# zhengchen1999/DOVE

Hardware: AMD Instinct MI355X
Metric: SR frames/s (33x720x1280 4x one-step, whole job) (higher is better)
Workload: dtype bf16; 1 GPU; synthetic 33x720x1280 HR clip (LR 180x320, 4x), one-step t=399, CogVideoX1.5-5B VAE + 42-layer DiT random-init, 1 clip per GPU (BASELINE configs[1]); weight_sums=True, vae_streams=2, variant=headline (bf16)

## Files before the change

### dove_amd/csrc/igemm.hip

```cpp
#include "igemm_args.h"


template <int BN, int BK>
struct FastCfg {
  static constexpr int BM = 128;
  static constexpr int CPR = BK / 8;
  static constexpr int CPR_LOG = (BK == 64) ? 3 : 2;
  static constexpr int RPG = 256 / CPR;
  static constexpr int NA = BM / RPG;
  static constexpr int B_SLOTS = BN * CPR;
  static constexpr int NB = (B_SLOTS + 255) / 256;
  static constexpr int A_BYTES = BM * BK * 2, B_BYTES = BN * BK * 2, STAGE = A_BYTES + B_BYTES;
  static constexpr int WN = (BN >= 128) ? 2 : 1, WM = 4 / WN;
  static constexpr int PT = (BM / WM) / 32, CT = (BN / WN) / 32;
  static constexpr int KK = BK / 16;
};

template <int BN, int BK>
__global__ __launch_bounds__(256) void igemm_fast_kernel(const IgemmArgs a) {
  using Cf = FastCfg<BN, BK>;
  constexpr int NA = Cf::NA, NB = Cf::NB, PT = Cf::PT, CT = Cf::CT, KK = Cf::KK, STAGE = Cf::STAGE, A_BYTES = Cf::A_BYTES;
  extern __shared__ __attribute__((aligned(16))) char smem[];
  const int tid = threadIdx.x, lane = tid & 63;
  const int wave = __builtin_amdgcn_readfirstlane(tid >> 6);
// ... 1053 lines not shown
#pragma unroll 4
  for (int r = 0; r < smallk::ROWS; ++r) {
    const long long m = r0 + r;
    if (m >= M) break;
    uint32_t xr[16];
#pragma unroll
    for (int q = 0; q < 4; ++q) {
      const uint4 v = xs[wave * smallk::ROWS + r][q];
      xr[q * 4 + 0] = v.x; xr[q * 4 + 1] = v.y; xr[q * 4 + 2] = v.z; xr[q * 4 + 3] = v.w;
    }
    float acc[4] = {b[0], b[1], b[2], b[3]};
#pragma unroll
    for (int k = 0; k < 16; ++k)
#pragma unroll
      for (int j = 0; j < 4; ++j)
        acc[j] = __builtin_amdgcn_fdot2_f32_bf16(__builtin_bit_cast(v2bf, wr[j][k]), __builtin_bit_cast(v2bf, xr[k]), acc[j], false);
    uint2 o;
    o.x = pack_bf2(acc[0], acc[1]);
    o.y = pack_bf2(acc[2], acc[3]);
    *(uint2*)(out + m * ldo + n0) = o;
  }
}

enum ConvKernel { K_IGEMM = 0, K_IGEMM_FAST, K_HALO4X, K_HALO4X_UP, K_GEMM8P, K_SMALLK, K_HALO4X_SUB };
static const char* const kKernelNames[] = {"igemm_kernel", "igemm_fast_kernel", "conv3x3_halo4x_kernel", "conv3x3_halo4x_kernel", "gemm8p_kernel",
                                           "smallk_kernel", "conv3x3_halo4x_kernel"};

static inline int desc_nb(const dove_conv_desc* d) { return d->nb > 1 ? d->nb : 1; }

static ConvKernel select_kernel(const dove_conv_desc* d) {
  const long long M = (long long)desc_nb(d) * d->t_out * d->h_out * d->w_out;
  const bool frame_fits = (long long)d->h_in * d->w_in * d->cin * 2 < (1ll << 31);
  const bool plain_gemm = d->kt == 1 && d->kh == 1 && d->kw == 1 && d->stride == 1 && d->up == 0 && d->tmode == 0 &&
                          d->t_in == d->t_out && d->h_in == d->h_out && d->w_in == d->w_out && d->cout_pad % 128 == 0 && M >= 4096 &&
                          (long long)512 * d->cin * 2 < (1ll << 31);
  const bool pointwise = d->kt == 1 && d->kh == 1 && d->kw == 1 && d->stride == 1 && d->up == 0 && d->tmode == 0 && d->t_in == d->t_out &&
                         d->h_in == d->h_out && d->w_in == d->w_out;
  if (pointwise && d->cin == 32 && d->act == 0 && !d->resid && !d->gate && d->cout_store >= 128) return K_SMALLK;
  if (plain_gemm) {
    if (d->cout_pad % 256 == 0 && d->cout_store % 256 == 0 && d->cin % 128 == 0 && d->cin >= 256 && (long long)256 * d->cin * 2 < (1ll << 31) &&
        d->ldo < (1 << 20) && d->ldr < (1 << 20) && (d->act == 0 || d->act == 1))
      return K_GEMM8P;
  }
  const bool conv3 = d->kh == 3 && d->kw == 3 && d->stride == 1 && d->pad_h == 1 && d->pad_w == 1 && d->act == 0 && !d->gate &&
                     d->cout_pad % 128 == 0 && frame_fits;
  if (conv3) {
    const bool same = d->up == 0 && d->tmode == 0 && d->h_out == d->h_in && d->w_out == d->w_in && d->w_out >= 16 && d->h_out >= 16;
    const bool ups = d->up == 1 && d->kt == 1 && d->h_out == 2 * d->h_in && d->w_out == 2 * d->w_in && d->h_out >= 16 && d->w_out >= 32;
    const bool h4 = d->cout_store % 128 == 0 && d->cin % 64 == 0 && d->ldo < (1 << 20) && (!d->resid || d->ldr < (1 << 20));
    if (same && h4) return K_HALO4X;
    if (ups && h4 && d->w_sub && d->h_in >= 16 && d->w_in >= 32) return K_HALO4X_SUB;
    if (ups && h4) return K_HALO4X_UP;
  }
  const int BN = (d->cout_pad % 128 == 0) ? 128 : ((d->cout_pad % 64 == 0) ? 64 : 32);
  const bool fits = frame_fits && (long long)BN * d->cin * 2 < (1ll << 31);
  return (d->up == 0 && fits) ? K_IGEMM_FAST : K_IGEMM;
}

static bool desc_size_ok(const dove_conv_desc* d, const char* who) {
  if (d && d->struct_size == sizeof(dove_conv_desc) && d->reserved == 0) return true;
  if (d) dove_set_error("%s: dove_conv_desc.struct_size is %u, this library (ABI %d) expects %zu - the caller's binding was written "
                        "against another include/dove_hip.h", who, d->struct_size, DOVE_ABI_VERSION, sizeof(dove_conv_desc));
  else dove_set_error("%s: null descriptor", who);
  return false;
}
extern "C" const char* dove_conv_kernel_name(const dove_conv_desc* d) { return desc_size_ok(d, "conv_kernel_name") ? kKernelNames[select_kernel(d)] : ""; }

template <int BN, int BK>
static int launch_igemm_fast(const IgemmArgs& a, unsigned grid, hipStream_t s) {
  constexpr int lds = 2 * (128 * BK * 2 + BN * BK * 2);
  static PerDeviceOnce attr_set;
  if (auto once_ = attr_set.guard()) (void)hipFuncSetAttribute((const void*)igemm_fast_kernel<BN, BK>, hipFuncAttributeMaxDynamicSharedMemorySize, lds);
  hipLaunchKernelGGL((igemm_fast_kernel<BN, BK>), dim3(grid), dim3(256), lds, s, a);
  DOVE_CHECK_LAUNCH("dove_conv_igemm_bf16");
  return DOVE_OK;
}
// ... 62 lines not shown
  DOVE_CHECK_ARG(d->x && d->w && d->out, "conv_igemm: null pointer");
  DOVE_CHECK_ARG(d->cin % 32 == 0 && d->cin > 0, "conv_igemm: Cin (%d) must be a positive multiple of 32 (pad on pack)", d->cin);
  DOVE_CHECK_ARG(d->cout_pad % 32 == 0 && d->cout_pad > 0, "conv_igemm: Cout_pad (%d) must be a multiple of 32", d->cout_pad);
  DOVE_CHECK_ARG(d->cout_store % 4 == 0 && d->cout_store <= d->cout_pad && d->cout_store > 0, "conv_igemm: bad cout_store %d", d->cout_store);
  DOVE_CHECK_ARG(d->ldo % 4 == 0 && d->ldo >= d->cout_store, "conv_igemm: ldo (%lld) must be a multiple of 4 and >= cout_store", d->ldo);
  DOVE_CHECK_ARG(!d->resid || (d->ldr % 4 == 0 && d->ldr >= d->cout_store), "conv_igemm: bad ldr %lld", d->ldr);
  DOVE_CHECK_ARG(!d->gate || d->resid, "conv_igemm: gate needs resid");
  DOVE_CHECK_ARG(d->kt >= 1 && d->kt <= 3 && d->kh >= 1 && d->kw >= 1, "conv_igemm: bad kernel size");
  DOVE_CHECK_ARG(d->stride == 1 || d->stride == 2, "conv_igemm: stride must be 1 or 2");
  DOVE_CHECK_ARG(d->up == 0 || d->up == 1, "conv_igemm: up must be 0/1");
  DOVE_CHECK_ARG(d->kt == 1 || (d->tmode == 0 && d->t_in == d->t_out), "conv_igemm: causal temporal taps need t_in == t_out and tmode 0");
  DOVE_CHECK_ARG(d->t_out > 0 && d->h_out > 0 && d->w_out > 0 && d->t_in > 0 && d->h_in > 0 && d->w_in > 0, "conv_igemm: empty tensor");
  DOVE_CHECK_ARG(d->nb >= 0 && d->nb <= 4096 && (long long)desc_nb(d) * d->t_out < (1 << 20), "conv_igemm: bad instance count nb = %d", d->nb);
  DOVE_CHECK_ARG(d->cache_stride == 0 || (d->cache && d->cache_stride >= (long long)(d->kt - 1) * d->h_in * d->w_in * d->cin),
                 "conv_igemm: cache_stride (%lld) is smaller than one instance's cache", d->cache_stride);
  DOVE_CHECK_ARG(desc_nb(d) == 1 || !d->gate, "conv_igemm: nb > 1 is not combined with gate");
  DOVE_CHECK_ARG(d->reserved2 == 0 && d->tdup >= 0 && d->tdup <= 2, "conv_igemm: bad tdup %d", d->tdup);
  DOVE_CHECK_ARG(!d->tdup || (d->kt == 3 && d->w_pair), "conv_igemm: tdup declares frame pairs of a kt == 3 conv and needs w_pair");
  DOVE_CHECK_ARG(!d->tdup || d->cache || d->w_first, "conv_igemm: tdup without a conv cache needs w_first too (frames whose three taps read one frame)");
  DOVE_CHECK_ARG(d->tdup != 2 || !d->cache, "conv_igemm: tdup == 2 (first frame single) is the head of a clip: no conv cache");
  DOVE_CHECK_ARG(!d->gn_partial || dove_conv_gn_partial_rows(d) > 0,
                 "conv_igemm: gn_partial requested but this call does not dispatch to a kernel that fuses the statistics");
  const ConvKernel kern0 = select_kernel(d);
  DOVE_CHECK_ARG(!d->out_f32 || (kern0 == K_IGEMM_FAST && !d->resid && d->act == 0),
                 "conv_igemm: out_f32 is only implemented for plain convs that dispatch to igemm_fast_kernel");
  long long rows_main = 0;
  if (kern0 == K_GEMM8P && gemm_tail_split(d, &rows_main)) {
    dove_conv_desc m = *d, t = *d;
    m.w_in = m.w_out = (int)rows_main;
    const long long tail = (long long)d->w_out - rows_main;
    t.w_in = t.w_out = (int)tail;
    t.x = (const char*)d->x + rows_main * d->cin * 2;
    t.out = (char*)d->out + rows_main * d->ldo * 2;
    if (d->resid) t.resid = (const char*)d->resid + rows_main * d->ldr * 2;
    t.gate_split = d->gate_split > rows_main ? d->gate_split - rows_main : 0;
    const int rc = conv_dispatch(&m, stream, K_GEMM8P);
    return rc ? rc : conv_dispatch(&t, stream, K_IGEMM_FAST);
  }
  return conv_dispatch(d, stream, kern0);
}

static int conv_dispatch(const dove_conv_desc* d, void* stream, ConvKernel kern) {
  const bf16_t* zp = zero_page();
  DOVE_CHECK_ARG(zp, "conv_igemm: could not allocate the zero page");
  IgemmArgs a;
  a.x = (const bf16_t*)d->x; a.cache = (const bf16_t*)d->cache; a.w = (const bf16_t*)d->w;
  a.bias = d->bias; a.resid = (const bf16_t*)d->resid; a.gate = d->gate; a.out = (bf16_t*)d->out; a.zero = zp;
  const int nb = desc_nb(d);
  a.T_out = nb * d->t_out; a.H_out = d->h_out; a.W_out = d->w_out;
  a.T_in = nb * d->t_in; a.H_in = d->h_in; a.W_in = d->w_in;
  a.seg_out = d->t_out; a.seg_in = d->t_in;
  a.cache_bs = d->cache_stride ? d->cache_stride : (long long)(d->kt - 1) * d->h_in * d->w_in * d->cin;
  a.Cin = d->cin; a.Cout_pad = d->cout_pad; a.Cout_st = d->cout_store;
  a.kt = d->kt; a.kh = d->kh; a.kw = d->kw; a.stride = d->stride; a.pad_h = d->pad_h; a.pad_w = d->pad_w;
  a.up = d->up; a.tmode = d->tmode; a.act = d->act; a.ldo = d->ldo; a.ldr = d->ldr; a.gate_split = d->gate_split;
  a.gn_partial = nullptr; a.cpg_log = 0;
  a.w_first = nullptr;
  a.w_pair = nullptr; a.tdup = 0;
  a.sub = 0;
  a.out_f32 = d->out_f32;
  a.nt_out = 0;
  a.reserved = 0;
  hipStream_t s = (hipStream_t)stream;
  const long long M = (long long)nb * d->t_out * d->h_out * d->w_out;
  switch (kern) {
    case K_GEMM8P: {
      a.tiles_n = d->cout_pad / 256;
      a.nt_out = (long long)M * d->ldo * 2 > (256ll << 20);
      const long long nt = ((M + gemm4x::BM - 1) / gemm4x::BM) * a.tiles_n;
      DOVE_CHECK_ARG(nt > 0 && nt < (1ll << 31), "conv_igemm: grid too large");
      DOVE_CHECK_ARG(!(d->gate && d->act), "conv_igemm: gate with activation is not a path of the reference");
      const int cus = cu_count();
      const unsigned grid4 = nt > cus ? (unsigned)cus : (unsigned)nt;
      static PerDeviceOnce attr8;
      if (auto once_ = attr8.guard()) {
        (void)hipFuncSetAttribute((const void*)gemm8p_kernel<false, false>, hipFuncAttributeMaxDynamicSharedMemorySize, gemm8p::LDS_BYTES);
        (void)hipFuncSetAttribute((const void*)gemm8p_kernel<true, false>, hipFuncAttributeMaxDynamicSharedMemorySize, gemm8p::LDS_BYTES);
        (void)hipFuncSetAttribute((const void*)gemm8p_kernel<false, true>, hipFuncAttributeMaxDynamicSharedMemorySize, gemm8p::LDS_BYTES);
      }
      if (d->gate) hipLaunchKernelGGL((gemm8p_kernel<false, true>), dim3(grid4), dim3(512), gemm8p::LDS_BYTES, s, a, M);
      else if (d->act == 1) hipLaunchKernelGGL((gemm8p_kernel<true, false>), dim3(grid4), dim3(512), gemm8p::LDS_BYTES, s, a, M);
      else hipLaunchKernelGGL((gemm8p_kernel<false, false>), dim3(grid4), dim3(512), gemm8p::LDS_BYTES, s, a, M);
      DOVE_CHECK_LAUNCH("dove_conv_igemm_bf16(gemm8p)");
      return DOVE_OK;
    }
    case K_SMALLK: {
      dim3 grid((unsigned)((M + 4 * smallk::ROWS - 1) / (4 * smallk::ROWS)), (unsigned)((d->cout_store + 255) / 256));
      hipLaunchKernelGGL(smallk_kernel, grid, dim3(256), 0, s, a.x, a.w, a.bias, a.out, M, d->cout_store, d->ldo);
// ... 86 lines not shown
```

### dove_amd/csrc/igemm_args.h

```cpp
#pragma once
#include <stdlib.h>

#include <type_traits>

#include "common.h"
#include "../../include/dove_hip.h"

struct IgemmArgs {
  const bf16_t* x;
  const bf16_t* cache;
  const bf16_t* w;
  const float* bias;
  const bf16_t* resid;
  const float* gate;
  bf16_t* out;
  const bf16_t* zero;
  int T_out, H_out, W_out;
  int T_in, H_in, W_in;
  int Cin, Cout_pad, Cout_st;
  int kt, kh, kw, stride, pad_h, pad_w, up, tmode, act;
  long long ldo, ldr;
  long long gate_split;
  int tw_log2, tiles_w, tiles_h, tiles_n;
  int reserved;
// ... 51 lines not shown
  q.m0 = __builtin_amdgcn_readfirstlane((int)(group * GM + within % gm) * gemm4x::BM);
  q.n0 = __builtin_amdgcn_readfirstlane((int)(within / gm) * gemm4x::BN);
  return q;
}
__device__ __forceinline__ void g4_open_tile(G4State& s, const IgemmArgs& a, const G4Const& k, int id) {
  s.n_tile = id;
  s.n_on = id < k.ntiles;
  const G4Tile q = g4_decode(k, id);
  const long long left = k.M - q.m0;
  const int rows = left < gemm4x::BM ? (int)left : gemm4x::BM;
  s.a_base = a.x + (long long)q.m0 * k.K;
  s.w_base = a.w + (long long)q.n0 * k.K;
  s.a_nrec = s.n_on ? rows * k.K * 2 : 0;
  s.w_nrec = s.n_on ? gemm4x::BN * k.K * 2 : 0;
  s.n_k4 = 0;
  s.soff = 0;
}
__device__ __forceinline__ void g4_advance(G4State& s, const IgemmArgs& a, const G4Const& k) {
  if (++s.n_k4 == k.nk4) g4_open_tile(s, a, k, s.n_tile + k.G);
  s.soff = s.n_k4 * (4 * gemm4x::ROWB);
}

int launch_igemm_legacy(const IgemmArgs& a, unsigned grid, int BN, bool bk64, hipStream_t s);
```

### dove_amd/lib.py

```python
from __future__ import annotations

import ctypes as C
import os

import torch

_HERE = os.path.dirname(os.path.abspath(__file__))
LIB_PATH = os.path.join(_HERE, "libdove_hip.so")
_lib = None

F32, BF16, U8 = 0, 1, 2
METRIC_PSNR, METRIC_SSIM, METRIC_RGB_TO_Y = 1, 2, 4
COLORFIX_WAVELET, COLORFIX_ADAIN, COLORFIX_CLAMP = 1, 2, 1
YUV_444, YUV_422, YUV_420, YUV_MONO = 0, 1, 2, 3
YUV_SITING_LEFT, YUV_SITING_CENTRE = 0, 1
VIDEO_RGB_U8, VIDEO_YUV = 0, 1
RESIZE_BILINEAR, RESIZE_BICUBIC, RESIZE_AREA = 0, 1, 2
ACT_NONE, ACT_RELU, ACT_SIGMOID, ACT_TANH = 0, 1, 2, 3


class ConvDesc(C.Structure):
    _fields_ = [
        ("struct_size", C.c_uint), ("reserved", C.c_uint),
        ("x", C.c_void_p), ("cache", C.c_void_p), ("w", C.c_void_p), ("bias", C.c_void_p),
# ... 90 lines not shown
                ("stride", C.c_int), ("pool", C.c_int), ("relu", C.c_int), ("reserved2", C.c_int),
                ("ldx", C.c_longlong), ("ldr", C.c_longlong), ("ldo", C.c_longlong)]

    def __init__(self, *a, **k):
        super().__init__(*a, **k)
        self.struct_size = C.sizeof(ResnetConvF32Args)


class PreNoise(C.Structure):
    _fields_ = [("eps", C.c_void_p), ("eps_dtype", C.c_int), ("sqrt_alpha", C.c_float), ("sqrt_one_minus_alpha", C.c_float)]


OPT_VAE_TILING, OPT_VAE_SAMPLE_HEIGHT, OPT_VAE_SAMPLE_WIDTH, OPT_DIT_LINEAR_MXFP8, OPT_DIT_ATTN_MXFP8, OPT_WEIGHT_SUMS, OPT_VAE_STREAMS = 1, 2, 3, 4, 5, 6, 7
STAT_HALO_PREPOSTED, STAT_HALO_BLOCKING, STAT_HALO_SENT, STAT_HALO_COMMUNICATORS = 100, 101, 102, 103


_VP, _I, _LL, _F = C.c_void_p, C.c_int, C.c_longlong, C.c_float
_ULL, _PI, _PLL = C.c_ulonglong, C.POINTER(C.c_int), C.POINTER(C.c_longlong)
XFER_FN = C.CFUNCTYPE(C.c_int, C.c_void_p, C.c_int, C.c_void_p, C.c_size_t, C.c_void_p)
GROUP_FN = C.CFUNCTYPE(C.c_int, C.c_void_p, C.c_void_p)

SIGNATURES = {
    "dove_conv_igemm_bf16": [C.POINTER(ConvDesc), _VP],
    "dove_groupnorm_stats_bf16": [_VP, _LL, _LL, _I, _F, _VP, _I, _VP, _VP],
    "dove_groupnorm_finalize_partials": [_VP, _LL, C.c_double, _F, _VP, _VP, _VP],
    "dove_groupnorm_stats_nb_bf16": [_VP, _I, _LL, _LL, _I, _F, _VP, _I, _VP, _VP],
    "dove_groupnorm_finalize_partials_nb": [_VP, _LL, _I, C.c_double, _F, _VP, C.c_size_t, _VP, _VP],
    "dove_groupnorm_apply_nb_bf16": [_VP, _VP, _I, _I, _I, _I, _I, _VP, _VP, _VP, _I, _VP, _I, _I, _I, _I, C.POINTER(C.c_int), _VP],
    "dove_avgpool_time_nb_bf16": [_VP, _I, _I, _LL, _VP, _VP],
    "dove_groupnorm_sums_bf16": [_VP, _LL, _LL, _I, _VP, _I, _VP, _VP],
    "dove_groupnorm_finalize_sums": [_VP, C.c_double, _F, _VP, _VP],
    "dove_groupnorm_sums_from_partials": [_VP, _LL, _VP, _VP, _VP],
    "dove_groupnorm_apply_bf16": [_VP, _VP, _I, _I, _I, _I, _VP, _VP, _VP, _I, _VP, _I, _I, _I, C.POINTER(C.c_int), _VP],
    "dove_layernorm_modulate_bf16": [_VP, _VP, _LL, _I, _F, _VP, _VP, _VP, _LL, _VP],
    "dove_qkv_post_bf16": [_VP, _LL, _LL, _I, _I, _I, _VP, _VP, _VP, _VP, _VP, _VP, _F, _F, _VP, _VP, _VP, _I, _VP, _VP],
    "dove_vt_quad_swap_bf16": [_VP, _LL, _LL, _VP],
    "dove_ulysses_place_bf16": [_VP, _VP, _VP, C.POINTER(C.c_longlong), _I, _I, _LL, _LL, _VP, _VP, _VP, _VP, _VP],
    "dove_cl_im2col3x3_from_ncthw": [_VP, _I, _I, _I, _I, _I, _I, _F, _F, _VP, _VP],
    "dove_conv_out_gather": [_VP, _LL, _I, _I, _I, _I, _VP, _F, _F, _F, _F, _VP, _I, _VP],
    "dove_attention_fwd_bf16": [_VP, _VP, _VP, _VP, _LL, _LL, _I, _I, _LL, _VP, _VP],
    "dove_qkv_post_mxfp8": [_VP, _LL, _LL, _I, _I, _I, _VP, _VP, _VP, _VP, _VP, _VP, _F, _F, _VP, _VP, _VP, _VP, _VP],
    "dove_attention_fwd_mxfp8": [_VP, _VP, _VP, _VP, _VP, _LL, _LL, _I, _I, _LL, _VP],
    "dove_cl_from_ncthw": [_VP, _I, _I, _LL, _I, _F, _F, _VP, _VP],
    "dove_ncthw_from_cl": [_VP, _LL, _I, _LL, _F, _F, _F, _F, _VP, _I, _VP],
    "dove_avgpool_time_bf16": [_VP, _I, _LL, _VP, _VP],
    "dove_posterior_sample": [_VP, _LL, _I, _LL, _VP, _I, _VP, _I, _VP],
# ... 91 lines not shown
    "dove_swin3d_window_gather_f32": [_VP, _I, _PI, _I, _PI, _PI, _VP, _VP],
    "dove_swin3d_window_scatter_f32": [_VP, _VP, _I, _PI, _I, _PI, _PI, _VP, _VP],
    "dove_swin3d_patch_merge_f32": [_VP, _LL, _I, _I, _I, _VP, _VP],
    "dove_swin3d_window_attention_f32": [_VP, _VP, _VP, _LL, _LL, _I, _I, _F, _VP, _VP, _I, _VP, _VP, _VP, _I, _VP, _LL, _VP],
    "dove_vqa_head_f64": [_VP, _LL, _I, _I, _I, _VP, _VP, _I, _VP, _VP, _VP, _VP],
    "dove_dwconv3d_f32": [_VP, _I, _I, _I, _I, _I, _VP, _VP, _VP, _VP],
    "dove_vqa_resized_view_f32": [C.POINTER(ImageView), _I, _I, _I, _VP, _I, _VP, _VP, _I, _VP, _VP, _I, _I, _I, C.POINTER(C.c_double),
                                  C.POINTER(C.c_double), _I, _VP, _VP],
    "dove_bmm_f32": [_VP, _LL, _LL, _VP, _LL, _LL, _VP, _VP, _LL, _LL, _VP, _LL, _LL, _I, _I, _I, _I, _F, _I, _VP],
    "dove_softmax_rows_f32": [_VP, _LL, _LL, _I, _VP, _LL, _VP],
    "dove_window_attention_f32": [_VP, _VP, _VP, _LL, _LL, _I, _I, _I, _F, _VP, _I, _VP, _VP, _I, _VP, _LL, _VP],
    "dove_maniqa_crops_f32": [C.POINTER(ImageView), _I, _I, _I, _I, _VP, _I, _I, _I, _VP, _VP],
    "dove_maniqa_tokens_f32": [_VP, _VP, _VP, _LL, _I, _I, _VP, _VP],
    "dove_mix_f32": [_VP, _LL, _LL, _VP, _LL, _LL, _F, _I, _I, _I, _I, _VP, _LL, _LL, _VP],
    "dove_maniqa_score": [_VP, _LL, _I, _I, _I, _I, _VP, _VP, _VP, _VP, _VP, _VP, _VP],
    "dove_png_encode": [C.POINTER(ImageView), _I, _I, _I, _I, _VP, C.c_size_t, _VP, _VP, _VP],
    "dove_zlib_huffman": [_VP, _LL, _LL, _VP, C.c_size_t, _VP, _VP, _VP],
    "dove_jpeg_encode": [C.POINTER(ImageView), _I, _I, _I, C.POINTER(C.c_int), _I, _VP, C.c_size_t, _VP, _VP, _VP],
}
PLAIN = {"dove_last_error": (C.c_char_p, []), "dove_abi_version": (C.c_int, []), "dove_comm_destroy": (None, [C.c_void_p]),
         "dove_conv_gn_partial_rows": (C.c_longlong, [C.POINTER(ConvDesc)]),
         "dove_conv_kernel_name": (C.c_char_p, [C.POINTER(ConvDesc)]),
         "dove_conv_partial_launches": (C.c_int, [C.POINTER(ConvDesc)]),
         "dove_attention_head_paths": (C.c_int, [C.POINTER(C.c_float), _I, C.POINTER(C.c_int)]),
         "dove_attention_path_name": (C.c_char_p, [_I]),
         "dove_device_info": (C.c_int, [_I, C.c_char_p, _I, C.POINTER(C.c_int), C.POINTER(C.c_longlong)]),
         "dove_destroy": (None, [_VP]),
         "dove_vae_decode_num_frames": (C.c_int, [_VP, _I]),
         "dove_get_option": (C.c_longlong, [_VP, _I]),
         "dove_comm_useful_ranks": (C.c_int, [_VP, _I, _I]),
         "dove_workspace_bytes": (C.c_size_t, [_VP, _I, _I, _I]),
         "dove_workspace_high_water": (C.c_size_t, [_VP]),
         "dove_fr_metrics_workspace_bytes": (C.c_size_t, [_I, _I, _I]),
         "dove_color_fix_workspace_bytes": (C.c_size_t, [_I, _I, _I, _I]),
         "dove_yuv_frame_bytes": (C.c_size_t, [_I, _I, _I]),
         "dove_poisson_noise_workspace_bytes": (C.c_size_t, [_I]),
         "dove_jpeg_roundtrip_workspace_bytes": (C.c_size_t, [_I, _I, _I]),
         "dove_vcodec_workspace_bytes": (C.c_size_t, [_I, _I, _I, _I]),
         "dove_vcodec_tools_workspace_bytes": (C.c_size_t, [_I, _I, _I, _I, _I]),
         "dove_chunk_planner_need": (C.c_longlong, [_VP]),
         "dove_chunk_planner_destroy": (None, [_VP]),
         "dove_video_workspace_bytes": (C.c_size_t, [_VP, C.POINTER(VideoParams)]),
         "dove_video_close": (None, [_VP]),
         "dove_instance_norm_f32_workspace_bytes": (C.c_size_t, [_I, _I, _I, _I]),
         "dove_flow_warp_error_workspace_bytes": (C.c_size_t, [_I, _I, _I]),
         "dove_convnet_conv_f32_kernel_name": (C.c_char_p, [C.POINTER(ConvnetConvF32Args)]),
# ... 90 lines not shown
```

### dove_amd/ops.py

```python
from __future__ import annotations

import ctypes as C
import math
from dataclasses import dataclass

import numpy as np
import torch

from . import lib as L


def _ru(x: int, m: int) -> int:
    return (x + m - 1) // m * m


@dataclass
class PackedConv:
    w: torch.Tensor
    bias: torch.Tensor | None
    kt: int
    kh: int
    kw: int
    cin: int
    cin_pad: int
# ... 55 lines not shown
        return [("w012", 0)] if tl == 0 else [("w01", 0), ("w2", 1)]
    if tdup == 1:
        if not cached and tl < 2:
            return [("w012", tl)]
        return [("w0", tl - 2), ("w12", tl)] if tl & 1 else [("w01", tl - 1), ("w2", tl)]
    if tl == 0:
        return [("w012", 0)]
    return [("w01", tl - 1), ("w2", tl)] if tl & 1 else [("w0", tl - 2), ("w12", tl)]


def temporal_groups(tl: int, tdup: int, cached: bool) -> int:
    return len(temporal_split(tl, tdup, cached))


_profiler = None


def set_profiler(records: list | None):
    global _profiler
    _profiler = records


def conv_kernel_name(x_shape, pc: PackedConv, *, stride=1, pad=(None, None), up=0, tmode=0, t_out=None, hw_out=None, act=0, gated=False,
                     resid=False, nb=1, partial=False):
    T, H, W, Cx = x_shape
    d = L.ConvDesc()
    d.nb = nb
    ph = (pc.kh - 1) // 2 if pad[0] is None else pad[0]
    pw = (pc.kw - 1) // 2 if pad[1] is None else pad[1]
    t_out = T if t_out is None else t_out
    if hw_out is None:
        hw_out = (H << up, W << up) if stride == 1 else ((H + 1 - pc.kh) // stride + 1, (W + 1 - pc.kw) // stride + 1)
    d.t_in, d.h_in, d.w_in, d.cin = T, H, W, Cx
    d.t_out, d.h_out, d.w_out = t_out, hw_out[0], hw_out[1]
    d.cout_pad, d.cout_store = pc.cout_pad, pc.cout_store
    d.kt, d.kh, d.kw, d.stride, d.pad_h, d.pad_w = pc.kt, pc.kh, pc.kw, stride, ph, pw
    d.up, d.tmode, d.act = up, tmode, act
    d.ldo = pc.cout_store
    d.ldr = pc.cout_store if resid else 0
    d.resid = 1 if (resid or gated) else None
    d.w_sub = 1 if (up == 1 and pc.kt == 1 and pc.kh == 3 and pc.kw == 3) else None
    d.gate = 1 if gated else None
    if partial:
        return int(L.load().dove_conv_partial_launches(C.byref(d)))
    return L.load().dove_conv_kernel_name(C.byref(d)).decode()


def conv(x: torch.Tensor, pc: PackedConv, *, cache: torch.Tensor | None = None, stride: int = 1, pad=(None, None),
         up: int = 0, tmode: int = 0, t_out: int | None = None, hw_out=None, resid: torch.Tensor | None = None,
         gate: torch.Tensor | None = None, gate_split: int = 0, act: int = 0, ldo: int | None = None,
         out: torch.Tensor | None = None,
         gn_eps: float | None = None, out_f32: bool = False, nb: int = 1, tdup: int = 0, weight_sums: bool = True) -> torch.Tensor:
    L.require_cuda(x, resid, gate, out)
    assert x.dtype == torch.bfloat16 and x.dim() == 4, (x.dtype, x.shape)
    T, H, W, Cx = x.shape
    assert T % nb == 0, (T, nb)
    T //= nb
    if Cx != pc.cin_pad:
        raise RuntimeError(f"conv: input has {Cx} channels, packed weight expects {pc.cin_pad}")
    ph = (pc.kh - 1) // 2 if pad[0] is None else pad[0]
    pw = (pc.kw - 1) // 2 if pad[1] is None else pad[1]
    if t_out is None:
        t_out = T
    if hw_out is None:
        hw_out = (H << up, W << up) if stride == 1 else ((H + 1 - pc.kh) // stride + 1, (W + 1 - pc.kw) // stride + 1)
    if ldo is None:
        ldo = pc.cout_store
    odt = torch.float32 if out_f32 else torch.bfloat16
    if out is None:
        out = torch.empty(nb * t_out, hw_out[0], hw_out[1], ldo, dtype=odt, device=x.device)
    else:
        assert out.shape == (nb * t_out, hw_out[0], hw_out[1], ldo) and out.dtype == odt
    cache_stride = 0
    if cache is not None:
        if nb > 1:
# ... 18 lines not shown
    d.out = out.data_ptr()
    d.t_in, d.h_in, d.w_in, d.cin = T, H, W, Cx
    d.t_out, d.h_out, d.w_out = t_out, hw_out[0], hw_out[1]
    d.cout_pad, d.cout_store = pc.cout_pad, pc.cout_store
    d.kt, d.kh, d.kw, d.stride, d.pad_h, d.pad_w = pc.kt, pc.kh, pc.kw, stride, ph, pw
    d.up, d.tmode, d.act = up, tmode, act
    d.ldo = ldo
    d.ldr = resid.shape[-1] if resid is not None else 0
    d.gate_split = gate_split
    d.out_f32 = int(out_f32)
    if resid is not None:
        assert resid.dtype == torch.bfloat16 and resid.numel() == nb * t_out * hw_out[0] * hw_out[1] * resid.shape[-1]
    if gate is not None:
        assert gate.dtype == torch.float32 and gate.shape == (2, pc.cout_pad)
    partial = None
    if gn_eps is not None and ldo == pc.cout_store:
        rows = int(L.load().dove_conv_gn_partial_rows(C.byref(d)))
        if rows > 0:
            partial = torch.empty(rows, 64, dtype=torch.float32, device=x.device)
            d.gn_partial = partial.data_ptr()
    if _profiler is not None:
        e0, e1 = torch.cuda.Event(enable_timing=True), torch.cuda.Event(enable_timing=True)
        e0.record()
    L.check(L.load().dove_conv_igemm_bf16(C.byref(d), L.stream_ptr()), "dove_conv_igemm_bf16")
    if _profiler is not None:
        e1.record()
        flops = 2.0 * nb * t_out * hw_out[0] * hw_out[1] * pc.cout * pc.cin * pc.kt * pc.kh * pc.kw
        name = L.load().dove_conv_kernel_name(C.byref(d)).decode()
        real = flops
        if name == "conv3x3_halo4x_kernel":
            if d.tdup and pc.kt == 3 and up == 0:
                real = flops * sum(temporal_groups(tl, d.tdup, cache is not None) for tl in range(t_out)) / (3.0 * t_out)
            elif d.w_first and pc.kt == 3 and up == 0:
                real = flops * (1.0 - (2.0 + (1.0 if t_out > 1 else 0.0)) / (3.0 * t_out))
            elif d.w_sub and up == 1 and H >= 16 and W >= 32:
                real = flops * 4.0 / 9.0
        _profiler.append(((pc.cin, pc.cout, pc.kt * pc.kh * pc.kw), flops, e0, e1, name, real))
    if partial is None:
        if getattr(out, "gn_stats", None) is not None:
            out.gn_stats = None
            out.gn_rows = None
    else:
        count = float(t_out * hw_out[0] * hw_out[1]) * (pc.cout_store // 32)
        if nb > 1:
            stats = torch.empty(nb, 32, 2, dtype=torch.float32, device=x.device)
            ws = _ws(x.device, nb * 512)
            L.check(L.load().dove_groupnorm_finalize_partials_nb(partial.data_ptr(), partial.shape[0] // nb, nb, count, gn_eps, L.ptr(ws),
                                                                 ws.numel() * 4, L.ptr(stats), L.stream_ptr()), "dove_groupnorm_finalize_partials_nb")
        else:
            stats = torch.empty(32, 2, dtype=torch.float32, device=x.device)
            L.check(L.load().dove_groupnorm_finalize_partials(partial.data_ptr(), partial.shape[0], count, gn_eps, L.ptr(_ws(x.device)),
# ... 1638 lines not shown
```

### include/dove_hip.h

```cpp
#ifndef DOVE_HIP_H
#define DOVE_HIP_H

#include <stddef.h>

#ifdef __cplusplus
extern "C" {
#endif

#define DOVE_ABI_VERSION 15

#define DOVE_F32 0
#define DOVE_BF16 1

const char* dove_last_error(void);
int dove_abi_version(void);
int dove_device_info(int dev, char* name, int name_len, int* cu_count, long long* total_mem);

typedef struct dove_conv_desc {
  unsigned int struct_size;
  unsigned int reserved;
  const void* x;
  const void* cache;
  const void* w;
  const float* bias;
  const void* resid;
  const float* gate;
  void* out;
  int t_in, h_in, w_in, cin;
  int t_out, h_out, w_out, cout_pad, cout_store;
  int kt, kh, kw, stride, pad_h, pad_w, up, tmode, act;
  long long ldo, ldr, gate_split;
  float* gn_partial;
  int out_f32;
  int nb;
  long long cache_stride;
  const void* w_first;
  const void* w_sub;
  const void* w_pair;
  int tdup;
  int reserved2;
} dove_conv_desc;
int dove_conv_igemm_bf16(const dove_conv_desc* d, void* stream);
const char* dove_conv_kernel_name(const dove_conv_desc* d);
int dove_conv_partial_launches(const dove_conv_desc* d);
long long dove_conv_gn_partial_rows(const dove_conv_desc* d);
int dove_groupnorm_finalize_partials(const float* partial, long long rows, double count, float eps, void* ws, float* stats,
                                     void* stream);

int dove_groupnorm_stats_bf16(const void* x, long long npix, long long frame_pix, int C, float eps, void* partial_ws, int ws_blocks,
                              float* stats, void* stream);
int dove_groupnorm_sums_bf16(const void* x, long long npix, long long frame_pix, int C, void* partial_ws, int ws_blocks, double* sums,
                             void* stream);
int dove_groupnorm_finalize_sums(const double* sums, double count, float eps, float* stats, void* stream);
int dove_groupnorm_sums_from_partials(const float* partial, long long rows, void* ws, double* sums, void* stream);
int dove_groupnorm_apply_bf16(const void* x, void* y, int T, int H, int W, int C, const float* stats,
                              const float* gamma, const float* beta, int silu, const void* yb, int hz, int wz,
                              int sshift, const int* tmap, void* stream);

int dove_groupnorm_stats_nb_bf16(const void* x, int nb, long long npix, long long frame_pix, int C, float eps, void* partial_ws,
                                 int ws_blocks, float* stats, void* stream);
int dove_groupnorm_finalize_partials_nb(const float* partial, long long rows, int nb, double count, float eps, void* ws, size_t ws_bytes,
                                        float* stats, void* stream);
int dove_groupnorm_apply_nb_bf16(const void* x, void* y, int nb, int T, int H, int W, int C, const float* stats, const float* gamma,
                                 const float* beta, int silu, const void* yb, int Tz, int hz, int wz, int sshift, const int* tmap,
                                 void* stream);
int dove_avgpool_time_nb_bf16(const void* x, int nb, int T, long long frame_elems, void* y, void* stream);
// ... 399 lines not shown
```

Measured before the change: 34.83 frames/s.

## Add persistent weight-stationary pointwise conv kernel for narrow-channel 1x1 convs

Adds a persistent streaming kernel for 1x1 (and kt=3 temporal 1x1) convolutions with small channel counts (Cin 32/128/256, Cout 32/128/256). It keeps the whole weight in LDS, double-buffers pixel loads through buffer loads, and uses MFMA 16x16x32 bf16. select_kernel routes matching large shapes to it instead of igemm_fast, which retiles weights for every tile and is suited to wide-channel GEMMs. It also exposes a direct entry point with a grid override and allows out_f32 on this path. The routing adds dispatch complexity and a risk of lower occupancy from the large LDS footprint.

```diff
diff --git a/dove_amd/csrc/igemm.hip b/dove_amd/csrc/igemm.hip
--- a/dove_amd/csrc/igemm.hip
+++ b/dove_amd/csrc/igemm.hip
@@ -1099,11 +1099,25 @@
   }
 }
 
-enum ConvKernel { K_IGEMM = 0, K_IGEMM_FAST, K_HALO4X, K_HALO4X_UP, K_GEMM8P, K_SMALLK, K_HALO4X_SUB };
+enum ConvKernel { K_IGEMM = 0, K_IGEMM_FAST, K_HALO4X, K_HALO4X_UP, K_GEMM8P, K_SMALLK, K_HALO4X_SUB, K_POINTWISE };
 static const char* const kKernelNames[] = {"igemm_kernel", "igemm_fast_kernel", "conv3x3_halo4x_kernel", "conv3x3_halo4x_kernel", "gemm8p_kernel",
-                                           "smallk_kernel", "conv3x3_halo4x_kernel"};
+                                           "smallk_kernel", "conv3x3_halo4x_kernel", "pointwise_stream_kernel"};
 
 static inline int desc_nb(const dove_conv_desc* d) { return d->nb > 1 ? d->nb : 1; }
+
+static bool pointwise_serves(const dove_conv_desc* d) {
+  if (!(d->kh == 1 && d->kw == 1 && d->stride == 1 && d->pad_h == 0 && d->pad_w == 0 && d->up == 0 && d->tmode == 0 && (d->kt == 1 || d->kt == 3) &&
+        d->t_in == d->t_out && d->h_in == d->h_out && d->w_in == d->w_out && d->act == 0 && !d->resid && !d->gate))
+    return false;
+  if (!(d->cin == 32 || d->cin == 128 || (d->cin == 256 && d->kt == 1))) return false;
+  if (!(d->cout_pad == 32 || d->cout_pad == 128 || (d->cout_pad == 256 && d->cin == 128 && d->kt == 1))) return false;
+  if (d->cin == 32 && d->cout_pad != 128) return false;
+  if (d->out_f32 && d->cout_pad != 32) return false;
+  if (!d->out_f32 && d->cout_store % 8) return false;
+  return (long long)d->h_in * d->w_in * d->cin * 2 < (1ll << 31) && d->ldo < (1 << 20) &&
+         (long long)desc_nb(d) * d->t_out * ((long long)d->h_out * d->w_out / 64 + 1) < (1ll << 30);
+}
+constexpr long long kPointwiseMinRows = 256ll * 4 * 64;
 
 static ConvKernel select_kernel(const dove_conv_desc* d) {
   const long long M = (long long)desc_nb(d) * d->t_out * d->h_out * d->w_out;
@@ -1129,6 +1143,7 @@
     if (ups && h4 && d->w_sub && d->h_in >= 16 && d->w_in >= 32) return K_HALO4X_SUB;
     if (ups && h4) return K_HALO4X_UP;
   }
+  if (pointwise_serves(d) && d->cin <= 128 && M >= kPointwiseMinRows) return K_POINTWISE;
   const int BN = (d->cout_pad % 128 == 0) ? 128 : ((d->cout_pad % 64 == 0) ? 64 : 32);
   const bool fits = frame_fits && (long long)BN * d->cin * 2 < (1ll << 31);
   return (d->up == 0 && fits) ? K_IGEMM_FAST : K_IGEMM;
@@ -1237,8 +1252,8 @@
   DOVE_CHECK_ARG(!d->gn_partial || dove_conv_gn_partial_rows(d) > 0,
                  "conv_igemm: gn_partial requested but this call does not dispatch to a kernel that fuses the statistics");
   const ConvKernel kern0 = select_kernel(d);
-  DOVE_CHECK_ARG(!d->out_f32 || (kern0 == K_IGEMM_FAST && !d->resid && d->act == 0),
-                 "conv_igemm: out_f32 is only implemented for plain convs that dispatch to igemm_fast_kernel");
+  DOVE_CHECK_ARG(!d->out_f32 || ((kern0 == K_IGEMM_FAST || kern0 == K_POINTWISE) && !d->resid && d->act == 0),
+                 "conv_igemm: out_f32 is only implemented for plain convs that dispatch to igemm_fast_kernel or pointwise_stream_kernel");
   long long rows_main = 0;
   if (kern0 == K_GEMM8P && gemm_tail_split(d, &rows_main)) {
     dove_conv_desc m = *d, t = *d;
@@ -1255,7 +1270,35 @@
   return conv_dispatch(d, stream, kern0);
 }
 
-static int conv_dispatch(const dove_conv_desc* d, void* stream, ConvKernel kern) {
+static int conv_dispatch(const dove_conv_desc* d, void* stream, ConvKernel kern, int pw_grid);
+static int conv_dispatch(const dove_conv_desc* d, void* stream, ConvKernel kern) { return conv_dispatch(d, stream, kern, 0); }
+
+extern "C" int dove_conv_pointwise_bf16(const dove_conv_desc* d, int grid, void* stream) {
+  if (!desc_size_ok(d, "conv_pointwise")) return DOVE_EINVAL;
+  DOVE_CHECK_ARG(d->x && d->w && d->out, "conv_pointwise: null pointer");
+  DOVE_CHECK_ARG(d->cout_store % 4 == 0 && d->cout_store <= d->cout_pad && d->cout_store > 0, "conv_pointwise: bad cout_store %d", d->cout_store);
+  DOVE_CHECK_ARG(d->ldo % 4 == 0 && d->ldo >= d->cout_store, "conv_pointwise: ldo (%lld) must be a multiple of 4 and >= cout_store", d->ldo);
+  DOVE_CHECK_ARG(d->t_out > 0 && d->h_out > 0 && d->w_out > 0, "conv_pointwise: empty tensor");
+  DOVE_CHECK_ARG(d->nb >= 0 && d->nb <= 4096 && (long long)desc_nb(d) * d->t_out < (1 << 20), "conv_pointwise: bad instance count nb = %d", d->nb);
+  DOVE_CHECK_ARG(d->cache_stride == 0 || (d->cache && d->cache_stride >= (long long)(d->kt - 1) * d->h_in * d->w_in * d->cin),
+                 "conv_pointwise: cache_stride (%lld) is smaller than one instance's cache", d->cache_stride);
+  DOVE_CHECK_ARG(grid >= 0 && grid <= 65536, "conv_pointwise: bad grid %d", grid);
+  DOVE_CHECK_ARG(!d->gn_partial, "conv_pointwise: the kernel does not fuse the GroupNorm statistics");
+  DOVE_CHECK_ARG(pointwise_serves(d), "conv_pointwise: not a shape pointwise_stream_kernel computes (see pointwise_serves in csrc/igemm.hip)");
+  return conv_dispatch(d, stream, K_POINTWISE, grid);
+}
+
+extern "C" long long dove_pointwise_weight_slot(int cin, int cout_pad, int kt, int slot) {
+  if (!((cin == 32 || cin == 128 || (cin == 256 && kt == 1)) && (kt == 1 || kt == 3) && (cout_pad == 32 || cout_pad == 128 || cout_pad == 256)) ||
+      (cin == 32 && cout_pad != 128) || (cout_pad == 256 && !(cin == 128 && kt == 1)))
+    return -1;
+  const int S = cin == 256 ? 4 : cin / 32, nseg = kt * cin / (32 * S);
+  if (slot < 0 || slot >= kt * cin * cout_pad / 8) return -1;
+  const PwSlot q = pw_weight_slot(S, cout_pad, nseg, cin, slot);
+  return ((long long)q.tap * cout_pad + q.ch) * cin + q.kin;
+}
+
+static int conv_dispatch(const dove_conv_desc* d, void* stream, ConvKernel kern, int pw_grid) {
   const bf16_t* zp = zero_page();
   DOVE_CHECK_ARG(zp, "conv_igemm: could not allocate the zero page");
   IgemmArgs a;
@@ -1279,6 +1322,7 @@
   hipStream_t s = (hipStream_t)stream;
   const long long M = (long long)nb * d->t_out * d->h_out * d->w_out;
   switch (kern) {
+    case K_POINTWISE: return launch_pointwise(a, cu_count(), pw_grid, s);
     case K_GEMM8P: {
       a.tiles_n = d->cout_pad / 256;
       a.nt_out = (long long)M * d->ldo * 2 > (256ll << 20);
diff --git a/dove_amd/csrc/igemm_args.h b/dove_amd/csrc/igemm_args.h
--- a/dove_amd/csrc/igemm_args.h
+++ b/dove_amd/csrc/igemm_args.h
@@ -97,3 +97,20 @@
 }
 
 int launch_igemm_legacy(const IgemmArgs& a, unsigned grid, int BN, bool bk64, hipStream_t s);
+struct PwSlot { int ch, tap, kin; };
+__host__ __device__ inline PwSlot pw_weight_slot(int S, int CP, int nseg, int cin, int idx) {
+  const int CH = CP < 128 ? CP : 128, NBLK = CH / 16, CPL = 4 * NBLK;
+  const int l = idx & 63;
+  int r = idx >> 6;
+  const int b = r % NBLK; r /= NBLK;
+  const int s = r % S; r /= S;
+  const int seg = r % nseg, h = r / nseg;
+  const int m = l & 15;
+  const int kg = seg * 32 * S + 32 * s + 8 * (l >> 4);
+  PwSlot q;
+  q.ch = h * CH + CPL * (m >> 2) + 4 * b + (m & 3);
+  q.tap = kg / cin;
+  q.kin = kg - q.tap * cin;
+  return q;
+}
+int launch_pointwise(const IgemmArgs& a, int cus, int grid, hipStream_t s);
diff --git a/dove_amd/csrc/pointwise.hip b/dove_amd/csrc/pointwise.hip
--- /dev/null
+++ b/dove_amd/csrc/pointwise.hip
@@ -0,0 +1,173 @@
+#include "igemm_args.h"
+
+namespace pointwise {
+constexpr int PIX = 64;
+constexpr int LDS_MAX = 64 * 1024 + 1024;
+constexpr int waves_per_simd(int S, int CP) { return (CP < 128 ? CP : 128) + 32 * S + 50 <= 256 ? 2 : 1; }
+}
+
+__device__ __forceinline__ void pw_store16(const u32x4 v, __amdgpu_buffer_rsrc_t srd, unsigned off) {
+  __builtin_amdgcn_raw_buffer_store_b128(v, srd, (int)off, 0, 0);
+  __builtin_amdgcn_sched_barrier(0);
+  asm volatile("s_nop 3" ::: "memory");
+  __builtin_amdgcn_sched_barrier(0);
+}
+
+template <int S, int CP, bool F32, int NSEG>
+__global__ __launch_bounds__(256, pointwise::waves_per_simd(S, CP)) void pointwise_stream_kernel(const IgemmArgs a, const int bpf, const int nitems) {
+  constexpr int CH = CP < 128 ? CP : 128;
+  constexpr int NH = CP / CH;
+  constexpr int NBLK = CH / 16;
+  constexpr int CPL = 4 * NBLK;
+  constexpr int SEG = 32 * S;
+  extern __shared__ __attribute__((aligned(16))) char smem[];
+  const int tid = threadIdx.x, lane = tid & 63;
+  const int wave = __builtin_amdgcn_readfirstlane(tid >> 6);
+  const int p = lane & 15, g = lane >> 4;
+  constexpr int nseg = NSEG;
+  const int HW = a.H_out * a.W_out;
+
+  const int nfrag = NH * nseg * S * NBLK * 64;
+  for (int idx = tid; idx < nfrag; idx += 256) {
+    const PwSlot q = pw_weight_slot(S, CP, nseg, a.Cin, idx);
+    *(uint4*)(smem + idx * 16) = *(const uint4*)(a.w + ((long long)q.tap * a.Cout_pad + q.ch) * a.Cin + q.kin);
+  }
+  float* const bias_l = (float*)(smem + nfrag * 16);
+  for (int c = tid; c < CP; c += 256) bias_l[c] = (a.bias && c < a.Cout_st) ? a.bias[c] : 0.f;
+  __syncthreads();
+
+  const long long frame_elems = (long long)HW * a.Cin;
+  const int stride = (int)gridDim.x * 4;
+  const int gw = (int)blockIdx.x * 4 + wave;
+
+  auto issue = [&](bf16x8 (&x)[S][4], int it, int seg) {
+    const bool live = it < nitems;
+    if (!live) it = 0;
+    const int bi = it / a.T_out, tt = it - bi * a.T_out;
+    const int koff = a.kt > 1 ? 0 : seg * SEG;
+    const bf16_t* fp = igemm_src_frame(a, tt, a.kt > 1 ? seg : 0, frame_elems) + koff;
+    const auto srd = __builtin_amdgcn_make_buffer_rsrc((void*)fp, (short)0, live ? (int)((frame_elems - koff) * 2) : 0, 0x00020000);
+#pragma unroll
+    for (int j = 0; j < 4; ++j) {
+      const int r = bi * pointwise::PIX + j * 16 + p;
+      const unsigned voff = r < HW ? (unsigned)((r * a.Cin + 8 * g) * 2) : 0x80000000u;
+#pragma unroll
+      for (int s = 0; s < S; ++s) x[s][j] = __builtin_bit_cast(bf16x8, __builtin_amdgcn_raw_buffer_load_b128(srd, (int)voff, s * 64, 0));
+    }
+  };
+
+  f32x4 acc[NBLK][4];
+  auto compute = [&](const bf16x8 (&x)[S][4], int c_it, int c_seg) {
+#pragma unroll
+    for (int h = 0; h < NH; ++h) {
+      if (c_seg == 0 || NH > 1) {
+#pragma unroll
+        for (int b = 0; b < NBLK; ++b)
+#pragma unroll
+          for (int j = 0; j < 4; ++j) acc[b][j] = f32x4{0.f, 0.f, 0.f, 0.f};
+      }
+      const char* wl = smem + (((h * nseg + c_seg) * S) * NBLK * 64 + lane) * 16;
+#pragma unroll
+      for (int s = 0; s < S; ++s)
+#pragma unroll
+        for (int b = 0; b < NBLK; ++b) {
+          const bf16x8 wf = *(const bf16x8*)(wl + (s * NBLK + b) * 1024);
+#pragma unroll
+          for (int j = 0; j < 4; ++j) acc[b][j] = __builtin_amdgcn_mfma_f32_16x16x32_bf16(wf, x[s][j], acc[b][j], 0, 0, 0);
+        }
+      if (c_seg != nseg - 1) continue;
+      const int bi = c_it / a.T_out, tt = c_it - bi * a.T_out;
+      const long long pix0 = (long long)tt * HW + (long long)bi * pointwise::PIX;
+      const int left = HW - bi * pointwise::PIX, npx = left < pointwise::PIX ? left : pointwise::PIX;
+      const int es = F32 ? 4 : 2;
+      void* ob = F32 ? (void*)((float*)a.out + pix0 * a.ldo) : (void*)(a.out + pix0 * a.ldo);
+      const auto srd_o = __builtin_amdgcn_make_buffer_rsrc(ob, (short)0, (int)(npx * a.ldo * es), 0x00020000);
+      const int c0 = h * CH + CPL * g;
+#pragma unroll
+      for (int j = 0; j < 4; ++j) {
+        const int q = j * 16 + p;
+        const unsigned obase = (unsigned)((q * a.ldo + c0) * es);
+        const bool okp = q < npx;
+        if (F32) {
+#pragma unroll
+          for (int b = 0; b < NBLK; ++b) {
+            f32x4 v = acc[b][j];
+            v += *(const f32x4*)(bias_l + c0 + 4 * b);
+            const bool ok = okp && c0 + 4 * b + 4 <= a.Cout_st;
+            pw_store16(__builtin_bit_cast(u32x4, v), srd_o, ok ? obase + 16 * b : 0x80000000u);
+          }
+        } else {
+#pragma unroll
+          for (int b = 0; b < NBLK; b += 2) {
+            f32x4 v0 = acc[b][j], v1 = acc[b + 1][j];
+            v0 += *(const f32x4*)(bias_l + c0 + 4 * b);
+            v1 += *(const f32x4*)(bias_l + c0 + 4 * b + 4);
+            const u32x4 v = {pack_bf2(v0[0], v0[1]), pack_bf2(v0[2], v0[3]), pack_bf2(v1[0], v1[1]), pack_bf2(v1[2], v1[3])};
+            const int c = c0 + 4 * b;
+            pw_store16(v, srd_o, (okp && c + 8 <= a.Cout_st) ? obase + 8 * b : 0x80000000u);
+          }
+        }
+      }
+    }
+  };
+
+  bf16x8 X[2][S][4];
+  int it = gw;
+  issue(X[0], it, 0);
+  __builtin_amdgcn_s_waitcnt(0x0F70);
+  while (it < nitems) {
+#pragma unroll
+    for (int seg = 0; seg < NSEG; ++seg) {
+      if (seg + 1 < NSEG) issue(X[(seg + 1) & 1], it, seg + 1);
+      else issue(X[NSEG & 1], it + stride, 0);
+      compute(X[seg & 1], it, seg);
+    }
+    if (NSEG & 1) {
+#pragma unroll
+      for (int s = 0; s < S; ++s)
+#pragma unroll
+        for (int j = 0; j < 4; ++j) X[0][s][j] = X[1][s][j];
+    }
+    it += stride;
+  }
+}
+
+template <int S, int CP, bool F32, int NSEG>
+static int pw_launch(const IgemmArgs& a, int bpf, int nitems, unsigned grid, hipStream_t s) {
+  const int lds = a.kt * a.Cin * CP * 2 + CP * 4;
+  static PerDeviceOnce attr_set;
+  if (auto once_ = attr_set.guard())
+    (void)hipFuncSetAttribute((const void*)pointwise_stream_kernel<S, CP, F32, NSEG>, hipFuncAttributeMaxDynamicSharedMemorySize, pointwise::LDS_MAX);
+  hipLaunchKernelGGL((pointwise_stream_kernel<S, CP, F32, NSEG>), dim3(grid), dim3(256), lds, s, a, bpf, nitems);
+  DOVE_CHECK_LAUNCH("dove_conv_igemm_bf16(pointwise)");
+  return DOVE_OK;
+}
+
+int launch_pointwise(const IgemmArgs& a, int cus, int grid, hipStream_t s) {
+  const int HW = a.H_out * a.W_out;
+  const int bpf = (HW + pointwise::PIX - 1) / pointwise::PIX;
+  const long long items = (long long)bpf * a.T_out;
+  DOVE_CHECK_ARG(items > 0 && items < (1ll << 30), "conv_igemm(pointwise): too many pixel blocks");
+  const long long wgs = (items + 3) / 4;
+  const long long want = grid > 0 ? grid : 2ll * cus;
+  const unsigned g = (unsigned)(wgs < want ? wgs : want);
+  const int nitems = (int)items;
+  const int S = a.Cin == 256 ? 4 : a.Cin / 32, nseg = a.kt * a.Cin / (32 * S);
+#define PW_FORM(S_, CP_, F32_, NSEG_) \
+  if (S == S_ && a.Cout_pad == CP_ && (a.out_f32 != 0) == F32_ && nseg == NSEG_) return pw_launch<S_, CP_, F32_, NSEG_>(a, bpf, nitems, g, s)
+  PW_FORM(1, 128, false, 3);
+  PW_FORM(1, 128, false, 1);
+  PW_FORM(4, 32, true, 3);
+  PW_FORM(4, 32, true, 1);
+  PW_FORM(4, 32, true, 2);
+  PW_FORM(4, 32, false, 1);
+  PW_FORM(4, 32, false, 2);
+  PW_FORM(4, 32, false, 3);
+  PW_FORM(4, 128, false, 1);
+  PW_FORM(4, 128, false, 2);
+  PW_FORM(4, 128, false, 3);
+  PW_FORM(4, 256, false, 1);
+#undef PW_FORM
+  dove_set_error("conv_igemm(pointwise): no instantiation for Cin %d, Cout_pad %d, out_f32 %d", a.Cin, a.Cout_pad, a.out_f32);
+  return DOVE_EINVAL;
+}
diff --git a/dove_amd/lib.py b/dove_amd/lib.py
--- a/dove_amd/lib.py
+++ b/dove_amd/lib.py
@@ -136,6 +136,7 @@
 
 SIGNATURES = {
     "dove_conv_igemm_bf16": [C.POINTER(ConvDesc), _VP],
+    "dove_conv_pointwise_bf16": [C.POINTER(ConvDesc), _I, _VP],
     "dove_groupnorm_stats_bf16": [_VP, _LL, _LL, _I, _F, _VP, _I, _VP, _VP],
     "dove_groupnorm_finalize_partials": [_VP, _LL, C.c_double, _F, _VP, _VP, _VP],
     "dove_groupnorm_stats_nb_bf16": [_VP, _I, _LL, _LL, _I, _F, _VP, _I, _VP, _VP],
@@ -273,6 +274,7 @@
          "dove_conv_gn_partial_rows": (C.c_longlong, [C.POINTER(ConvDesc)]),
          "dove_conv_kernel_name": (C.c_char_p, [C.POINTER(ConvDesc)]),
          "dove_conv_partial_launches": (C.c_int, [C.POINTER(ConvDesc)]),
+         "dove_pointwise_weight_slot": (C.c_longlong, [_I, _I, _I, _I]),
          "dove_attention_head_paths": (C.c_int, [C.POINTER(C.c_float), _I, C.POINTER(C.c_int)]),
          "dove_attention_path_name": (C.c_char_p, [_I]),
          "dove_device_info": (C.c_int, [_I, C.c_char_p, _I, C.POINTER(C.c_int), C.POINTER(C.c_longlong)]),
diff --git a/dove_amd/ops.py b/dove_amd/ops.py
--- a/dove_amd/ops.py
+++ b/dove_amd/ops.py
@@ -101,7 +101,7 @@
 
 
 def conv_kernel_name(x_shape, pc: PackedConv, *, stride=1, pad=(None, None), up=0, tmode=0, t_out=None, hw_out=None, act=0, gated=False,
-                     resid=False, nb=1, partial=False):
+                     resid=False, nb=1, partial=False, out_f32=False):
     T, H, W, Cx = x_shape
     d = L.ConvDesc()
     d.nb = nb
@@ -120,6 +120,7 @@
     d.resid = 1 if (resid or gated) else None
     d.w_sub = 1 if (up == 1 and pc.kt == 1 and pc.kh == 3 and pc.kw == 3) else None
     d.gate = 1 if gated else None
+    d.out_f32 = int(out_f32)
     if partial:
         return int(L.load().dove_conv_partial_launches(C.byref(d)))
     return L.load().dove_conv_kernel_name(C.byref(d)).decode()
@@ -129,7 +130,8 @@
          up: int = 0, tmode: int = 0, t_out: int | None = None, hw_out=None, resid: torch.Tensor | None = None,
          gate: torch.Tensor | None = None, gate_split: int = 0, act: int = 0, ldo: int | None = None,
          out: torch.Tensor | None = None,
-         gn_eps: float | None = None, out_f32: bool = False, nb: int = 1, tdup: int = 0, weight_sums: bool = True) -> torch.Tensor:
+         gn_eps: float | None = None, out_f32: bool = False, nb: int = 1, tdup: int = 0, weight_sums: bool = True,
+         pointwise_grid: int | None = None) -> torch.Tensor:
     L.require_cuda(x, resid, gate, out)
     assert x.dtype == torch.bfloat16 and x.dim() == 4, (x.dtype, x.shape)
     T, H, W, Cx = x.shape
@@ -194,11 +196,14 @@
     if _profiler is not None:
         e0, e1 = torch.cuda.Event(enable_timing=True), torch.cuda.Event(enable_timing=True)
         e0.record()
-    L.check(L.load().dove_conv_igemm_bf16(C.byref(d), L.stream_ptr()), "dove_conv_igemm_bf16")
+    if pointwise_grid is not None:
+        L.check(L.load().dove_conv_pointwise_bf16(C.byref(d), pointwise_grid, L.stream_ptr()), "dove_conv_pointwise_bf16")
+    else:
+        L.check(L.load().dove_conv_igemm_bf16(C.byref(d), L.stream_ptr()), "dove_conv_igemm_bf16")
     if _profiler is not None:
         e1.record()
         flops = 2.0 * nb * t_out * hw_out[0] * hw_out[1] * pc.cout * pc.cin * pc.kt * pc.kh * pc.kw
-        name = L.load().dove_conv_kernel_name(C.byref(d)).decode()
+        name = "pointwise_stream_kernel" if pointwise_grid is not None else L.load().dove_conv_kernel_name(C.byref(d)).decode()
         real = flops
         if name == "conv3x3_halo4x_kernel":
             if d.tdup and pc.kt == 3 and up == 0:
diff --git a/include/dove_hip.h b/include/dove_hip.h
--- a/include/dove_hip.h
+++ b/include/dove_hip.h
@@ -42,6 +42,8 @@
 } dove_conv_desc;
 int dove_conv_igemm_bf16(const dove_conv_desc* d, void* stream);
 const char* dove_conv_kernel_name(const dove_conv_desc* d);
+int dove_conv_pointwise_bf16(const dove_conv_desc* d, int grid, void* stream);
+long long dove_pointwise_weight_slot(int cin, int cout_pad, int kt, int slot);
 int dove_conv_partial_launches(const dove_conv_desc* d);
 long long dove_conv_gn_partial_rows(const dove_conv_desc* d);
 int dove_groupnorm_finalize_partials(const float* partial, long long rows, double count, float eps, void* ws, float* stats,
```

Result: no change. 34.86 frames/s (median of 6 runs) (+0.1%).
